# bolcom/serenade

Measured on AMD Instinct MI355X. Metric: predict_next queries/sec, higher is better.
Workload: dtype u32 ids / i32 accumulators / f64 scores; 1 GPU; BASELINE configs[2]: synthetic 60000000 interactions / 1760000 items, k=1500 m=2500 idf_weighting=2 last_items=4 how_many=21; batch_per_gpu=1048576, query_pool_batches=2, parallelism=query-sharded replicas x1 (no data-path collective), index=csr (built by this library)

## Files before the change

### serenade_amd/csrc/srn_fast.hip

```cpp
#include <hip/hip_runtime.h>

#include <cstdio>
#include <cstdlib>

#include "srn_device.h"
#include "srn_prep.h"
#include "srn_kernels.h"

namespace srn {

#ifndef SRN_FAST_NT
#define SRN_FAST_NT 1
#endif
typedef uint32_t fin_v4u __attribute__((ext_vector_type(4)));
__device__ __forceinline__ void fin_store(uint4* p, const uint4& v) {
#if SRN_FAST_NT
    __builtin_nontemporal_store((fin_v4u{v.x, v.y, v.z, v.w}), reinterpret_cast<fin_v4u*>(p));
#else
    *p = v;
#endif
}
__device__ __forceinline__ uint4 fin_load(const uint4* p) {
#if SRN_FAST_NT
    const fin_v4u v = __builtin_nontemporal_load(reinterpret_cast<const fin_v4u*>(p)); return make_uint4(v.x, v.y, v.z, v.w);
#else
    return *p;
#endif
}
template <typename T> __device__ __forceinline__ void row_store(T* p, T v) {
#if SRN_FAST_NT
    __builtin_nontemporal_store(v, p);
#else
    *p = v;
#endif
}

enum { FS_NB = 0, FS_FAIL, FS_SURV, FS_CCNT, FS_HITS, FS_LIVE, FS_SCAN_A = 8, FS_SCAN_B = 8, FS_W3 = 8, FS_CLS = 16, FS_TACC = 32 };
static constexpr uint32_t F_SIDF = F_LDS_BYTES, F_SATTR = F_SIDF + 512 * 8, F_TOTAL = F_SATTR + 512, F_SINV = F_W10 + 384;
static_assert(F_TOTAL * F_WG_PER_CU <= 160 * 1024, "LDS budget with the sample constants");

#ifndef SRN_FAST_RELOAD_ROWS
#define SRN_FAST_RELOAD_ROWS 0
#endif
#ifndef SRN_FAST_PRIO_LEVELS
#define SRN_FAST_PRIO_LEVELS 22201333
#endif
enum { FP_REC = 10000000, FP_FRONT = 1000000, FP_CUT = 100000, FP_REQ = 10000, FP_WALK = 1000, FP_HARV = 100, FP_WB = 10, FP_HAND = 1 };
#ifndef SRN_FAST_PRIO_X
#define SRN_FAST_PRIO_X 92
#endif
#define FAST_PRIO_X(div) do { if (SRN_FAST_PRIO_LEVELS && ((SRN_FAST_PRIO_X) / (div)) % 10 != 9) __builtin_amdgcn_s_setprio((short)(((SRN_FAST_PRIO_X) / (div)) % 10)); } while (0)
#ifndef SRN_MID_PRIO_LEVELS
#define SRN_MID_PRIO_LEVELS SRN_FAST_PRIO_LEVELS
#endif
#define FAST_PRIO(ph) do { if (SRN_FAST_PRIO_LEVELS) __builtin_amdgcn_s_setprio((short)((((MID) ? (SRN_MID_PRIO_LEVELS) : (SRN_FAST_PRIO_LEVELS)) / (ph)) % 10)); } while (0)
#ifndef SRN_FAST_STOP
#define SRN_FAST_STOP (-1)
#endif
#define FAST_TICK(ph) \
    do { if (ticking && tid == 0) { const long long t_ = clock64(); tacc[ph] += (unsigned long long)(t_ - t_prev); t_prev = t_; } } while (0); \
    if (SRN_FAST_STOP == (ph)) continue

__device__ __forceinline__ uint32_t fast_offset_of(uint32_t idx, uint64_t r) {
    if (idx < F_REP_ITEMS) return (F_DIRECT + idx * F_REP + ((uint32_t)r & (F_REP - 1u))) * 4u;
    return idx < F_DIRECT ? idx * 4u : (F_SKETCH - F_HOT) + (idx & (F_SK_WORDS - 1u)) * 4u;
}
#ifndef SRN_FAST_PHANTOM_OOR
#define SRN_FAST_PHANTOM_OOR 1
#endif
static constexpr uint32_t F_PHANTOM_WORDS = 256u;
static constexpr uint32_t F_PHANTOM = SRN_FAST_PHANTOM_OOR ? F_BIG_TOTAL - (F_TOTAL - F_SIDF) - 256u * 4u - F_M_MAX : F_DUMP;
static_assert(!SRN_FAST_PHANTOM_OOR || (F_PHANTOM >= F_TOTAL && F_PHANTOM % 4u == 0u), "the phantom words lie beyond the 53 KB forms' LDS allocation");
static_assert(F_PHANTOM + F_PHANTOM_WORDS * 4u - F_HOT <= 65536u, "16-bit row offsets");
static_assert(!SRN_FAST_PHANTOM_OOR || F_PHANTOM_WORDS * 4u <= F_M_MAX, "inside the numerator bytes' room");
__device__ __forceinline__ uint32_t fast_phantom(uint64_t r, uint32_t j) {
    return (F_PHANTOM - F_HOT) + ((((uint32_t)r * 0x9E3779B1u + j * 0x85EBCA6Bu) >> 21) & (F_PHANTOM_WORDS - 1u)) * 4u;
}
__global__ __launch_bounds__(1024) void rows_to_packed_kernel(const uint64_t* __restrict__ row_off, const uint32_t* __restrict__ row_items, uint64_t n,
                                                              const uint32_t* __restrict__ block_base, uint32_t* __restrict__ packed, uint32_t* __restrict__ ext16) {
    __shared__ uint32_t wave_tot[16];
    const uint64_t r = (uint64_t)blockIdx.x * 1024 + threadIdx.x;
    const int lane = threadIdx.x & 63, wave = threadIdx.x >> 6;
    uint64_t o = 0, len = 0;
    if (r < n) { o = row_off[r]; len = row_off[r + 1] - o; }
    const uint32_t e = len > 30 ? (uint32_t)((len - 28 + 7) / 8) : 0u;
    const uint32_t inc = wave_incl_scan(e);
    if (lane == 63) wave_tot[wave] = inc;
    __syncthreads();
    uint32_t base = block_base[blockIdx.x];
    for (int w = 0; w < wave; ++w) base += wave_tot[w];
    const uint32_t eblk = base + inc - e;
    if (r > n) return;
    const uint32_t inl = len > 30 ? 28u : (uint32_t)len;
    uint32_t sl[16];
    auto half = [&](uint32_t j) -> uint32_t { return j < inl ? fast_offset_of(row_items[o + j], r) : fast_phantom(r, j); };
    sl[0] = (uint32_t)(len > 0xFFFFu ? 0xFFFFu : len);
#pragma unroll
    for (uint32_t wd = 1; wd < 16; ++wd) sl[wd] = half(2 * wd - 2) | (half(2 * wd - 1) << 16);
    if (len > 30) {
        sl[15] = eblk;
        for (uint32_t b = 0; b < e; ++b) {
            uint32_t wv[4];
#pragma unroll
            for (uint32_t x = 0; x < 4; ++x) {
                const uint64_t j0 = 28 + 8ull * b + 2 * x;
                const uint32_t lo = j0 < len ? fast_offset_of(row_items[o + j0], r) : fast_phantom(r, (uint32_t)j0);
                const uint32_t hi = j0 + 1 < len ? fast_offset_of(row_items[o + j0 + 1], r) : fast_phantom(r, (uint32_t)j0 + 1);
                wv[x] = lo | (hi << 16);
            }
            reinterpret_cast<uint4*>(ext16)[(size_t)eblk + b] = make_uint4(wv[0], wv[1], wv[2], wv[3]);
        }
    }
    uint4* dst = reinterpret_cast<uint4*>(packed + r * 16);
#pragma unroll
    for (int qd = 0; qd < 4; ++qd) dst[qd] = make_uint4(sl[4 * qd], sl[4 * qd + 1], sl[4 * qd + 2], sl[4 * qd + 3]);
}

__global__ __launch_bounds__(1024) void rows_to_packed_frag_kernel(const uint64_t* __restrict__ row_off, const uint32_t* __restrict__ row_items, uint64_t n,
                                                                   const uint32_t* __restrict__ block_base, uint32_t* __restrict__ packed, uint32_t* __restrict__ ext16) {
    __shared__ uint32_t wave_tot[16];
    const uint64_t r = (uint64_t)blockIdx.x * 1024 + threadIdx.x;
    const int lane = threadIdx.x & 63, wave = threadIdx.x >> 6;
    uint64_t o = 0, len = 0;
    if (r < n) { o = row_off[r]; len = row_off[r + 1] - o; }
    const uint32_t e = len > 6 ? (uint32_t)((len - 4 + 7) / 8) : 0u;
    const uint32_t inc = wave_incl_scan(e);
    if (lane == 63) wave_tot[wave] = inc;
    __syncthreads();
    uint32_t base = block_base[blockIdx.x];
    for (int w = 0; w < wave; ++w) base += wave_tot[w];
    const uint32_t eblk = base + inc - e;
    if (r > n) return;
    const uint32_t inl = len > 6 ? 4u : (uint32_t)len;
    auto half = [&](uint32_t j) -> uint32_t { return j < inl ? fast_offset_of(row_items[o + j], r) : fast_phantom(r, j); };
    uint32_t sl[4];
    sl[0] = (uint32_t)(len > 0xFFFFu ? 0xFFFFu : len);
#pragma unroll
    for (uint32_t wd = 1; wd < 4; ++wd) sl[wd] = half(2 * wd - 2) | (half(2 * wd - 1) << 16);
    if (len > 6) {
        sl[3] = eblk;
        for (uint32_t b = 0; b < e; ++b) {
            uint32_t wv[4];
#pragma unroll
            for (uint32_t x = 0; x < 4; ++x) {
                const uint64_t j0 = 4 + 8ull * b + 2 * x;
                const uint32_t lo = j0 < len ? fast_offset_of(row_items[o + j0], r) : fast_phantom(r, (uint32_t)j0);
                const uint32_t hi = j0 + 1 < len ? fast_offset_of(row_items[o + j0 + 1], r) : fast_phantom(r, (uint32_t)j0 + 1);
                wv[x] = lo | (hi << 16);
            }
            reinterpret_cast<uint4*>(ext16)[(size_t)eblk + b] = make_uint4(wv[0], wv[1], wv[2], wv[3]);
        }
    }
    reinterpret_cast<uint4*>(packed)[r] = make_uint4(sl[0], sl[1], sl[2], sl[3]);
}

#ifndef SRN_MERGE_G
#define SRN_MERGE_G 8
#endif
__device__ __forceinline__ uint32_t merge_team(uint32_t total) {
    const uint32_t want = (total + (uint32_t)SRN_MERGE_G - 1u) / (uint32_t)SRN_MERGE_G;
    return want <= 64u ? 6u : want <= 128u ? 7u : want <= 256u ? 8u : 9u;
}
typedef __attribute__((address_space(3))) uint32_t lds_u32;
__device__ __forceinline__ uint32_t lds_addr(const uint32_t* p) { return (uint32_t)(uintptr_t)(const lds_u32*)p; }
__device__ __forceinline__ uint32_t lds_ld(uint32_t a) { return *(const lds_u32*)(uintptr_t)a; }
__device__ __forceinline__ void lds_st(uint32_t a, uint32_t v) { *(lds_u32*)(uintptr_t)a = v; }
__device__ __forceinline__ void merge_pair(const uint32_t* in, uint32_t* out, uint32_t sa, uint32_t la, uint32_t lb, uint32_t ttid, uint32_t lg_nthr) {
    if ((ttid >> lg_nthr) != 0u) return;
#ifndef SRN_MERGE_ODD
#define SRN_MERGE_ODD 1
#endif
    const uint32_t total = la + lb, g = ((total + (1u << lg_nthr) - 1u) >> lg_nthr) | (SRN_MERGE_ODD ? 1u : 0u);
    const uint32_t d0 = min(ttid * g, total), d1 = min(d0 + g, total);
    if (d0 >= d1) return;
    const uint32_t a0 = lds_addr(in) + sa * 4u;
    const uint32_t lo = d0 > lb ? d0 - lb : 0u, hi = min(d0, la);
    uint32_t p = a0 + lo * 4u - 4u;
    const uint32_t span = min(la, lb);
    if (span != 0u) {
        uint32_t xh = a0 + max(hi, 1u) * 4u - 4u, kb = d0 != 0u ? 2u * a0 + (la + d0) * 4u - 4u : 2u * a0;
        asm volatile("" : "+v"(xh), "+v"(kb));
        for (uint32_t st = 4u << (31u - (uint32_t)__clz((int)span)); st >= 4u; st >>= 1) {
            const uint32_t x = min(p + st, xh);
            p = lds_ld(x) > lds_ld(kb - x) ? x : p;
        }
    }
    uint32_t pa = p + 4u, pb = 2u * a0 + (la + d0) * 4u - 4u - p;
    uint32_t ea = a0 + la * 4u, eb = ea + lb * 4u;
    asm volatile("" : "+v"(ea), "+v"(eb));
    uint32_t va = 0u, vb = 0u;
    if (pa < ea) va = lds_ld(pa);
    if (pb < eb) vb = lds_ld(pb);
    uint32_t c = lds_addr(out) + (sa + d0) * 4u; const uint32_t ce = c + (d1 - d0) * 4u, ce1 = ce - 4u;
    auto put = [&](uint32_t off) {
        const bool ta = va > vb;
        lds_st(c + off, max(va, vb));
        const uint32_t q = (ta ? pa : pb) + 4u;
        pa = ta ? q : pa; pb = ta ? pb : q;
        const uint32_t nxt = lds_ld(q);
        const uint32_t nv = q < (ta ? ea : eb) ? nxt : 0u;
        va = ta ? nv : va; vb = ta ? vb : nv;
    };
    for (; c < ce1; c += 8u) { put(0u); put(4u); }
    if (c < ce) lds_st(c, max(va, vb));
}

#ifndef SRN_FAST_FUSED_CUT
#define SRN_FAST_FUSED_CUT 1
#endif
template <int G>
__device__ __forceinline__ uint32_t fast_cut(const uint32_t* F, uint32_t* nbl, uint32_t n, uint32_t NB, uint32_t m, uint32_t k, const uint8_t* wlut, uint32_t* misc, uint32_t tid, uint32_t lane) {
    constexpr int BLOCK = 512;
    const uint32_t NBM = (1u << NB) - 1u;
    const uint32_t g = (n + BLOCK - 1) / BLOCK, o0 = min(tid * g, n), o1 = min(o0 + g, n);
    uint32_t fv[G + 3];
#pragma unroll
    for (int x = 0; x < G + 3; ++x) fv[x] = F[min(o0 + (uint32_t)x, n - 1u)];
    const uint32_t prev0 = o0 > 0u && o0 < o1 ? F[o0 - 1u] >> NB : 0xFFFFFFFFu;
#pragma unroll
    for (int x = 0; x < G + 3; ++x) fv[x] = o0 + (uint32_t)x < n ? fv[x] : 0u;
    {
        uint32_t carry = 0u, carry_r = 0xFFFFFFFFu;
#pragma unroll
        for (int x = G + 2; x >= 0; --x) { const uint32_t r = fv[x] >> NB; carry = r == carry_r ? carry | fv[x] : fv[x]; carry_r = r; fv[x] = carry; }
    }
    uint32_t fmask = 0u, firsts = 0u;
    {
        uint32_t prev = prev0;
#pragma unroll
        for (int x = 0; x < G; ++x) { const bool in = o0 + (uint32_t)x < o1; const uint32_t r = fv[x] >> NB; const bool f1 = in && r != prev; fmask |= f1 ? 1u << x : 0u; firsts += f1; prev = in ? r : prev; }
    }
    uint32_t Call;
    const uint32_t idx0 = block_excl_scan<BLOCK>(firsts, misc + FS_SCAN_A, Call);
    const uint32_t Cm = min(Call, m);
    if (Cm <= k) {
        uint32_t idx = idx0;
#pragma unroll
        for (int x = 0; x < G; ++x) if ((fmask >> x) & 1u) { if (idx < m) nbl[idx] = fv[x]; ++idx; }
        return Cm;
    }
    uint32_t inm = 0u; unsigned long long nmp = 0ull, acc = 0ull;
    {
        uint32_t idx = idx0, nmv[G];
#pragma unroll
        for (int x = 0; x < G; ++x) nmv[x] = (uint32_t)wlut[fv[x] & NBM];
#pragma unroll
        for (int x = 0; x < G; ++x) {
            const bool f1 = (fmask >> x) & 1u, in = f1 && idx < m;
            idx += f1;
            inm |= in ? 1u << x : 0u;
            nmp |= in ? (unsigned long long)nmv[x] << (4 * x) : 0ull;
            acc += in ? 1ull << (4u * nmv[x]) : 0ull;
        }
    }
    uint32_t* cls = misc + FS_CLS;
    {
        const uint32_t wc = wave_class_counts(acc, lane);
        const uint32_t mycnt = lane < 16u ? wc : 0u;
        if (mycnt) atomicAdd(&cls[lane], mycnt);
    }
    __syncthreads();
    uint32_t nstar, rstar;
    {
        const uint32_t cv = lane < 16u ? cls[lane] : 0u; const uint32_t pre = wave_incl_scan(cv);
        const uint32_t suf = (uint32_t)__builtin_amdgcn_readlane((int)pre, 63) - pre + cv;
        const unsigned long long reach = __ballot(suf >= k);
        nstar = 63u - (uint32_t)__clzll((long long)reach);
        rstar = k - ((uint32_t)__builtin_amdgcn_readlane((int)suf, (int)nstar) - (uint32_t)__builtin_amdgcn_readlane((int)cv, (int)nstar));
    }
    uint32_t mine = 0;
#pragma unroll
    for (int x = 0; x < G; ++x) mine += ((inm >> x) & 1u) && (uint32_t)((nmp >> (4 * x)) & 15ull) == nstar;
    uint32_t tot_star;
    uint32_t before = block_excl_scan<BLOCK>(mine, misc + FS_SCAN_B, tot_star);
    uint32_t sel = 0, tmask = 0;
#pragma unroll
    for (int x = 0; x < G; ++x) {
        const bool in = (inm >> x) & 1u; const uint32_t c = (uint32_t)((nmp >> (4 * x)) & 15ull);
        const bool eq = in && c == nstar, take = in && (c > nstar || (eq && before < rstar));
        tmask |= take ? 1u << x : 0u; sel += take; before += eq;
    }
    const uint32_t inc = wave_incl_scan(sel);
    uint32_t base = 0; if (lane == 63u && inc) base = atomicAdd(&misc[FS_NB], inc);
    uint32_t at = (uint32_t)__builtin_amdgcn_readlane((int)base, 63) + inc - sel;
#pragma unroll
    for (int x = 0; x < G; ++x) if ((tmask >> x) & 1u) nbl[at++] = fv[x];
    return 0xFFFFFFFFu;
}

enum { FM_FUSED = 0, FM_FRONT = 1, FM_BACK = 2 };
template <int WG_PER_CU, bool FRAG, bool WIDE, int MODE = FM_FUSED, bool MID = false, bool BIG = false, bool LONG = false, bool TINY = false>
#ifndef SRN_FAST_WAVES
#define SRN_FAST_WAVES (WG_PER_CU * 2)
#endif
#ifndef SRN_TINY_WAVES
#define SRN_TINY_WAVES 2
#endif
__global__ __launch_bounds__(512, TINY ? SRN_TINY_WAVES : BIG ? 4 : SRN_FAST_WAVES) void vmis_fast_kernel(DeviceIndex ix_arg, LaunchParams p_arg, FastParams f_arg) {
#if SRN_FAST_SMALL
    static_assert(!BIG || MID, "BIG is a form of MID"); static_assert(!LONG || BIG, "LONG is a form of BIG");
    constexpr uint32_t SIDF = BIG ? F_BIG_TOTAL - (F_TOTAL - F_SIDF) : F_SIDF, SATTR = SIDF + 512 * 8;
    constexpr uint32_t MW = (SIDF - F_WORK) / 4;
    __shared__ __attribute__((aligned(16))) char smem[BIG ? F_BIG_TOTAL : F_TOTAL];
#else
    extern __shared__ __attribute__((aligned(16))) char smem[];
#endif
    typedef const __attribute__((address_space(4))) char* KArg;
    const KArg ka = (KArg)__builtin_amdgcn_kernarg_segment_ptr();
    constexpr size_t OFF_P = (sizeof(DeviceIndex) + alignof(LaunchParams) - 1) / alignof(LaunchParams) * alignof(LaunchParams);
    constexpr size_t OFF_F = (OFF_P + sizeof(LaunchParams) + alignof(FastParams) - 1) / alignof(FastParams) * alignof(FastParams);
    const __attribute__((address_space(4))) DeviceIndex& ix = *(const __attribute__((address_space(4))) DeviceIndex*)ka;
    const __attribute__((address_space(4))) LaunchParams& p = *(const __attribute__((address_space(4))) LaunchParams*)(ka + OFF_P);
    const __attribute__((address_space(4))) FastParams& f = *(const __attribute__((address_space(4))) FastParams*)(ka + OFF_F);
    constexpr int BLOCK = 512, NW = 8;
    constexpr int NL = LONG ? (int)F_LONG_LISTS : MID ? (int)F_MID_LISTS : 4;
    constexpr uint32_t SINV = F_SINV;
    static_assert(!MID || MODE == FM_FUSED, "MID: fused form only");
    const uint32_t tid = threadIdx.x, lane = tid & 63u, wave = tid >> 6;
    const unsigned long long lt = (1ull << lane) - 1ull;
// ... 347 lines not shown
            } else
                for (uint32_t o = o0; o < o1; ++o) { const uint32_t r = F[o] >> NB; firsts += r != prev; prev = r; }
            for (uint32_t i = tid; i < min(n, p.m); i += BLOCK) D[i] = 0;
            if (MID && tid < (LONG ? 256u : 64u)) cls_area[tid] = 0u;
            if constexpr (LONG) for (uint32_t i = tid; i < (min(n, p.m) + 3u) / 4u; i += BLOCK) dn_area[i] = 0u;
            uint32_t idx = block_excl_scan<BLOCK>(firsts, misc + FS_SCAN_A, Call);
            prev = prev0;
            if (g <= (uint32_t)MC_G) {
                uint32_t fv[MC_G];
#pragma unroll
                for (int x = 0; x < MC_G; ++x) fv[x] = F[min(o0 + (uint32_t)x, n - 1u)];
#pragma unroll
                for (int x = 0; x < MC_G; ++x) {
                    const bool in = o0 + (uint32_t)x < o1; const uint32_t r = fv[x] >> NB; const bool f1 = in && r != prev;
                    idx += f1; prev = in ? r : prev;
                    if constexpr (LONG) {
                        if (in && idx - 1u < p.m) { if (f1) D[idx - 1u] = fv[x]; atomicAdd(&dn_area[(idx - 1u) >> 2], (uint32_t)wlut[fv[x] & 31u] << (8u * ((idx - 1u) & 3u))); }
                    } else
                    if (in && idx - 1u < p.m) atomicOr(&D[idx - 1u], fv[x]);
                }
            } else
                for (uint32_t o = o0; o < o1; ++o) {
                    const uint32_t v = F[o], r = v >> NB; const bool f1 = r != prev;
                    idx += f1; prev = r;
                    if constexpr (LONG) { if (idx - 1u < p.m) { if (f1) D[idx - 1u] = v; atomicAdd(&dn_area[(idx - 1u) >> 2], (uint32_t)wlut[v & 31u] << (8u * ((idx - 1u) & 3u))); } }
                    else
                    if (idx - 1u < p.m) atomicOr(&D[idx - 1u], v);
                }
            Cm = min(Call, p.m);
        }
        __syncthreads();
        FAST_TICK(2);
        auto dn_of = [&](uint32_t i) -> uint32_t { return (dn_area[i >> 2] >> (8u * (i & 3u))) & 255u; };
        auto w_long = [&](uint32_t slot, uint32_t num) -> uint32_t { return (uint32_t)((9 - (int)(uint32_t)wlut[32u + (slot & 31u)]) * (int)num); };
        if (Cm <= p.k) {
            K = Cm;
            if constexpr (LONG) { for (uint32_t i = tid; i < Cm; i += BLOCK) { const uint32_t dvv = D[i]; nb2[i] = make_uint2(dvv, w_long(dvv, dn_of(i))); } __syncthreads(); }
        } else {
            uint32_t* cls = MID ? cls_area : misc + FS_CLS;
            const uint32_t g = (Cm + BLOCK - 1) / BLOCK, o0 = min(tid * g, Cm), o1 = min(o0 + g, Cm);
            uint32_t dv[5], nmv[5];
#pragma unroll
            for (int x = 0; x < 5; ++x) dv[x] = o0 + x < o1 ? D[o0 + x] : 0u;
#pragma unroll
            for (int x = 0; x < 5; ++x) { if constexpr (LONG) nmv[x] = o0 + x < o1 ? dn_of(o0 + (uint32_t)x) : 0u; else nmv[x] = o0 + x < o1 ? num_of(dv[x] & NBM) : 0u; }
            if constexpr (MID) {
#pragma unroll
                for (int x = 0; x < 5; ++x) if (o0 + x < o1) atomicAdd(&cls[nmv[x]], 1u);
            } else
            {
                unsigned long long acc = 0;
#pragma unroll
                for (int x = 0; x < 5; ++x) acc += o0 + x < o1 ? 1ull << (4u * nmv[x]) : 0ull;
                const uint32_t wc = wave_class_counts(acc, lane);
                const uint32_t mycnt = lane < 16u ? wc : 0u;
                if (mycnt) atomicAdd(&cls[lane], mycnt);
            }
            __syncthreads();
            uint32_t nstar, rstar;
            if constexpr (LONG) {
                const uint4 c4 = reinterpret_cast<const uint4*>(cls)[lane];
                const uint32_t s4 = c4.x + c4.y + c4.z + c4.w, pre4 = wave_incl_scan(s4);
                const uint32_t above = (uint32_t)__builtin_amdgcn_readlane((int)pre4, 63) - pre4;
                const uint32_t suf3 = above + c4.w, suf2 = suf3 + c4.z, suf1 = suf2 + c4.y, suf0 = suf1 + c4.x;
                const unsigned long long reach = __ballot(suf0 >= p.k);
                const int top = 63 - __clzll((long long)reach);
                const uint32_t jsel = suf3 >= p.k ? 3u : suf2 >= p.k ? 2u : suf1 >= p.k ? 1u : 0u;
                const uint32_t sufs = jsel == 3u ? suf3 : jsel == 2u ? suf2 : jsel == 1u ? suf1 : suf0, cnts = jsel == 3u ? c4.w : jsel == 2u ? c4.z : jsel == 1u ? c4.y : c4.x;
                nstar = (uint32_t)__builtin_amdgcn_readlane((int)(4u * lane + jsel), top);
                rstar = p.k - ((uint32_t)__builtin_amdgcn_readlane((int)sufs, top) - (uint32_t)__builtin_amdgcn_readlane((int)cnts, top));
            } else
            {
                const uint32_t cv = (MID || lane < 16u) ? cls[lane] : 0u; const uint32_t pre = wave_incl_scan(cv);
                const uint32_t suf = (uint32_t)__builtin_amdgcn_readlane((int)pre, 63) - pre + cv;
                const unsigned long long reach = __ballot(suf >= p.k);
                nstar = 63u - (uint32_t)__clzll((long long)reach);
                rstar = p.k - ((uint32_t)__builtin_amdgcn_readlane((int)suf, (int)nstar) - (uint32_t)__builtin_amdgcn_readlane((int)cv, (int)nstar));
            }
            uint32_t mine = 0;
#pragma unroll
            for (int x = 0; x < 5; ++x) mine += o0 + x < o1 && nmv[x] == nstar;
            uint32_t tot_star;
            uint32_t before = block_excl_scan<BLOCK>(mine, misc + FS_SCAN_B, tot_star);
            uint32_t sel = 0; bool take[5];
#pragma unroll
            for (int x = 0; x < 5; ++x) {
                const bool in_r = o0 + x < o1, eq = nmv[x] == nstar;
                take[x] = in_r && (nmv[x] > nstar || (eq && before < rstar));
                sel += take[x]; before += in_r && eq;
            }
            const uint32_t inc = wave_incl_scan(sel);
            uint32_t base = 0; if (lane == 63u && inc) base = atomicAdd(&misc[FS_NB], inc);
            uint32_t at = (uint32_t)__builtin_amdgcn_readlane((int)base, 63) + inc - sel;
#pragma unroll
            for (int x = 0; x < 5; ++x) if (take[x]) { if constexpr (LONG) nb2[at++] = make_uint2(dv[x], w_long(dv[x], nmv[x])); else nbl[at++] = dv[x]; }
            __syncthreads();
            K = misc[FS_NB];
        }
        }
        }

        FAST_TICK(4);
        if constexpr (SRN_FAST_ROW_PREFETCH == 2 && !MID && MODE == FM_FUSED && !FRAG) asm volatile("" :: "v"(pfv[0]), "v"(pfv[1]), "v"(pfv[2]), "v"(pfv[3]));
        FAST_PRIO(FP_REQ); FAST_PRIO_X(10);
        if constexpr (MODE == FM_FRONT) {
            if (tid == 0) xq[0] = K;
#pragma unroll
            for (int j = 0; j < 3; ++j) { const uint32_t e = tid + (uint32_t)j * BLOCK; if ((uint32_t)j * BLOCK < K && e < K) xq[1u + e] = nbl[e]; }
            continue;
        }

        uint32_t svr[3]; uint4 rq[3], rq1[3];
        uint32_t wvr[3] = {0u, 0u, 0u};
#pragma unroll
        for (int t = 0; t < 3; ++t) {
            const uint32_t j = wave * 64u + lane + (uint32_t)t * BLOCK;
            if constexpr (MODE == FM_BACK) svr[t] = j < K ? xsv[t] : 0u;
            else if constexpr (LONG) { const uint2 e2 = nb2[K ? min(j, K - 1u) : 0u]; svr[t] = K ? e2.x : 0u; wvr[t] = e2.y; }
            else
            svr[t] = K ? nbl[min(j, K - 1u)] : 0u;
            const size_t r = (MODE == FM_BACK ? j < K : K != 0u) ? (size_t)(base + (svr[t] >> NB)) : (size_t)n_kept;
            rq[t] = *reinterpret_cast<const uint4*>(&f.row_packed[r * (FRAG ? 1 : 4)]); rq1[t] = make_uint4(0u, 0u, 0u, 0u);
        }
        if (((SRN_FAST_PRIO_X) / 10) % 10 != 9) FAST_PRIO(FP_REQ);
        {
            uint4* z = reinterpret_cast<uint4*>(smem + F_HOT);
            for (uint32_t i = tid; i < (clr_lo - F_HOT) / 16u; i += BLOCK) z[i] = make_uint4(0u, 0u, 0u, 0u);
            if (tid < 64u) reinterpret_cast<uint4*>(thist)[tid] = make_uint4(0u, 0u, 0u, 0u);
            if (tid < F_TABLE_WORDS / 4u) { reinterpret_cast<uint4*>(ikeys)[tid] = make_uint4(EMPTY32, EMPTY32, EMPTY32, EMPTY32);
                                            reinterpret_cast<uint4*>(iacc)[tid] = make_uint4(0u, 0u, 0u, 0u); }
        }
        __syncthreads();
        FAST_PRIO(FP_WALK);
        FAST_TICK(8);
        auto add2 = [&](uint32_t wd, uint32_t w) {
            if constexpr (LONG) {
                const bool neg = (int)w < 0; const uint32_t a = wd & 0xFFFFu, b = wd >> 16;
                if (!neg || a < F_SKETCH - F_HOT) atomicAdd((uint32_t*)(acc_base + a), w);
                if (!neg || b < F_SKETCH - F_HOT) atomicAdd((uint32_t*)(acc_base + b), w);
            } else {
            atomicAdd((uint32_t*)(acc_base + (wd & 0xFFFFu)), w); atomicAdd((uint32_t*)(acc_base + (wd >> 16)), w); } };
        constexpr uint32_t INL1 = FRAG ? 6u : 14u, INL2 = FRAG ? 20u : 28u;
        uint32_t cnt3 = 0;
#pragma unroll
        for (int t = 0; t < 3; ++t) {
            const bool m3 = wave * 64u + lane + (uint32_t)t * BLOCK < K && (rq[t].x & 0xFFFFu) > INL1;
            const unsigned long long b3 = __ballot(m3);
            if (m3) nbl[qpos(cnt3 + (uint32_t)__popcll(b3 & lt))] = LONG ? wave * 64u + lane + (uint32_t)t * BLOCK : svr[t];
            cnt3 += (uint32_t)__popcll(b3);
        }
#ifdef SRN_FAST_SUBTICKS
        FAST_TICK(5);
#endif
        if constexpr (!FRAG) {
#pragma unroll
            for (int t = 0; t < 3; ++t) {
                const bool more6 = wave * 64u + lane + (uint32_t)t * BLOCK < K && (rq[t].x & 0xFFFFu) > 6u;
                const size_t r1 = more6 ? (size_t)(base + (svr[t] >> NB)) : (size_t)n_kept;
                rq1[t] = *reinterpret_cast<const uint4*>(&f.row_packed[r1 * 4 + 1]);
            }
        }
        auto tok_slot = [&](uint32_t tok) -> uint32_t { if constexpr (LONG) return nb2[tok].x; else return tok; };
        auto tok_w = [&](uint32_t tok, uint32_t slot) -> uint32_t { if constexpr (LONG) return nb2[tok].y; else return w10_of(slot & NBM); };
        auto q3_load = [&](uint32_t p0, uint32_t& tok, uint32_t& sv, uint32_t& hdr, uint4& c4, uint4& d4, uint32_t& blk) {
            tok = nbl[qpos(min(p0 + lane, cnt3 - 1u))];
            sv = tok_slot(tok);
            if constexpr (FRAG) {
                const uint4 s4 = *reinterpret_cast<const uint4*>(f.row_packed + (size_t)(base + (sv >> NB)));
                hdr = s4.x;
                const uint4* eb = reinterpret_cast<const uint4*>(f.row_ext16) + ((hdr & 0xFFFFu) > 6u ? (size_t)s4.w : (size_t)0);
                c4 = eb[0]; d4 = eb[1]; blk = s4.w + 2u;
            } else {
                const RowQuad* rowp = f.row_packed + (size_t)(base + (sv >> NB)) * 4;
                hdr = *reinterpret_cast<const uint32_t*>(rowp); c4 = *reinterpret_cast<const uint4*>(rowp + 2); d4 = *reinterpret_cast<const uint4*>(rowp + 3); blk = d4.w;
            } };
        uint32_t tk3 = 0, sv3 = 0, hdr3 = 0, blk3 = 0; uint4 c43 = make_uint4(0u, 0u, 0u, 0u), d43 = c43;
        if (cnt3) q3_load(0u, tk3, sv3, hdr3, c43, d43, blk3);
        const uint32_t qn = MID ? q_after : ordered || listed ? q_ord_next : q + gridDim.x;
        const bool park = MID ? q_after != 0xFFFFFFFFu : ordered || listed ? q_ord_next != 0xFFFFFFFFu : qn < p.nq;
        if (wave == 1u && park) {
            const char* const rn = p.prep + (size_t)qn * p.prep_stride + lane * 4u;
            if (lane * 4u < p.prep_stride) __builtin_amdgcn_global_load_lds((const __attribute__((address_space(1))) void*)rn, (__attribute__((address_space(3))) void*)pre, 4, 0, 0);
            if (256u + lane * 4u < min(p.prep_stride, 320u)) __builtin_amdgcn_global_load_lds((const __attribute__((address_space(1))) void*)(rn + 256), (__attribute__((address_space(3))) void*)(pre + 64), 4, 0, 0);
        }
#pragma unroll
        for (int t = 0; t < 3; ++t) {
            if (wave * 64u + (uint32_t)t * BLOCK < K) {
                const bool act = wave * 64u + lane + (uint32_t)t * BLOCK < K;
                const uint32_t w = LONG ? wvr[t] : w10_of(svr[t] & NBM), len = rq[t].x & 0xFFFFu;
                if constexpr (FRAG) { if (act) { add2(rq[t].y, w); add2(rq[t].z, w); if (len <= 6u) add2(rq[t].w, w); } }
                else {
                if (act) { add2(rq[t].y, w); add2(rq[t].z, w); add2(rq[t].w, w); }
                if (act && len > 6u) { add2(rq1[t].x, w); add2(rq1[t].y, w); add2(rq1[t].z, w); add2(rq1[t].w, w); }
                }
            }
        }
        auto add_tail = [&](uint32_t p0, uint32_t tok, uint32_t sv, uint32_t hdr, const uint4& c4, const uint4& d4, uint32_t blk) {
            const bool act = p0 + lane < cnt3;
            const uint32_t len = hdr & 0xFFFFu, w = tok_w(tok, sv);
            const bool more = FRAG ? true : len > 30u;
            if constexpr (FRAG) {
                if (act) { add2(c4.x, w); add2(c4.y, w); add2(c4.z, w); add2(c4.w, w); }
                if (act && len > 12u) { add2(d4.x, w); add2(d4.y, w); add2(d4.z, w); add2(d4.w, w); }
            } else if (act) {
                add2(c4.x, w); add2(c4.y, w); add2(c4.z, w); add2(c4.w, w);
                add2(d4.x, w); add2(d4.y, w); add2(d4.z, w);
                if (len <= 30u) add2(d4.w, w);
            }
            for (uint32_t t8 = INL2; __ballot(act && more && t8 < len) != 0ull; t8 += 8u) {
                if (act && more && t8 < len) {
                    const uint4 e4 = reinterpret_cast<const uint4*>(f.row_ext16)[(size_t)blk + ((t8 - INL2) >> 3)];
                    add2(e4.x, w); add2(e4.y, w); add2(e4.z, w); add2(e4.w, w);
                }
            } };
#ifdef SRN_FAST_SUBTICKS
        FAST_TICK(6);
#endif
        FAST_PRIO_X(1);
        if (cnt3) add_tail(0u, tk3, sv3, hdr3, c43, d43, blk3);
        for (uint32_t p0 = 64u; p0 < cnt3; p0 += 64u) { uint32_t tk, sv, hdr, blk; uint4 c4, d4; q3_load(p0, tk, sv, hdr, c4, d4, blk); add_tail(p0, tk, sv, hdr, c4, d4, blk); }
#ifdef SRN_FAST_SUBTICKS
        FAST_TICK(7);
#endif
        __syncthreads();
        FAST_PRIO(FP_HARV);
        FAST_TICK(9);
        uint32_t t32m1; uint32_t floor_b;
        {
            const uint32_t e = lane * NW + wave;
            uint32_t v = hot[e];
            if (F_REP_ITEMS && e < F_REP_ITEMS) {
                const uint4* rp = reinterpret_cast<const uint4*>(hot + F_DIRECT + e * F_REP);
                const uint4 a = rp[0], b = rp[1];
                v = a.x + a.y + a.z + a.w + b.x + b.y + b.z + b.w;
            }
            if (!SRN_FAST_PHANTOM_OOR || BIG)
            for (uint32_t i = tid; i < F_PHANTOM_WORDS; i += BLOCK) ((uint32_t*)(smem + F_PHANTOM))[i] = 0u;
            bool valid = (LONG ? (int)v > 0 : v != 0u) && e != cur_idx;
            double x = 0.0; uint32_t tie = 0;
            tie = f.meta_sample[tid].id_rank;
            if (business) valid = valid && business_ok(cur_attr, (uint32_t)((const uint8_t*)(smem + SATTR))[tid]);
            if (valid) x = ((const double*)(smem + SIDF))[tid] * (double)v;
            const uint32_t k32 = (uint32_t)((unsigned long long)__double_as_longlong(x) >> 32);
            {
                uint32_t vv = k32, third = 0;
#pragma unroll
                for (int t = 0; t < 3; ++t) {
                    const uint32_t mx = wave_max(vv);
                    third = mx;
                    const unsigned long long bal = __ballot(vv == mx);
                    if ((int)lane == __ffsll((long long)bal) - 1) vv = 0;
                }
                for (uint32_t t = 3u; t < ((p.how_many + 7u) >> 3); ++t) {
                    const uint32_t mx = wave_max(vv);
                    third = mx;
                    const unsigned long long bal = __ballot(vv == mx);
                    if ((int)lane == __ffsll((long long)bal) - 1) vv = 0;
                }
                if (lane == 0u) misc[FS_W3 + wave] = third;
            }
            __syncthreads();
            uint32_t t32 = 0xFFFFFFFFu;
#pragma unroll
            for (int w = 0; w < NW; ++w) t32 = min(t32, misc[FS_W3 + w]);
            t32m1 = t32 ? t32 - 1u : 0u;
            const bool take = valid && k32 >= t32m1;
            const uint32_t at = wave_append(take, &misc[FS_CCNT]);
            if (take) { if (at < F_CAND_CAP) { ckey[at] = (unsigned long long)__double_as_longlong(x); cidx[at] = tie; } else misc[FS_FAIL] = 1;
                        const uint32_t hb = k32 >> 16, tb = t32 >> 16; if (t32) atomicAdd(&thist[hb > tb ? min(hb - tb, 255u) : 0u], 1u); }
            const double x_lo = __longlong_as_double((long long)((unsigned long long)t32m1 << 32));
            const double inv = ((const double*)(smem + SINV))[min(lane, 8u)];
            const uint32_t my_floor = (uint32_t)fmin(4.0e9, fmax(1.0, floor(x_lo * inv * (1.0 - 1e-9)) - 1.0));
            floor_b = (uint32_t)__builtin_amdgcn_readlane((int)my_floor, 8);
            {
                const uint32_t wv = (uint32_t)__builtin_amdgcn_readfirstlane((int)wave);
                const uint4* h4 = reinterpret_cast<const uint4*>(hot);
                static_assert(F_HOT_WORDS == 4096 || F_HOT_WORDS == 3840, "quads per thread below (3840: the 40 KB timing experiment)");
                constexpr uint32_t NQ2 = F_HOT_WORDS / 4u - 128u - (uint32_t)BLOCK;
                const uint4 a4 = h4[128u + tid];
                const uint4 b4 = tid < NQ2 ? h4[128u + (uint32_t)BLOCK + tid] : make_uint4(0u, 0u, 0u, 0u);
                if (tid == NQ2 - 1u) hot[F_HOT_WORDS - 1u] = 0u;
                const uint32_t fl1 = (uint32_t)__builtin_amdgcn_readlane((int)my_floor, (int)(1u + (wv >> 1)));
                const uint32_t fl2 = (uint32_t)__builtin_amdgcn_readlane((int)my_floor, (int)min(5u + (wv >> 1), 7u));
                auto quad = [&](const uint4& q4, uint32_t e0, uint32_t fl) {
                    const uint32_t mx = LONG ? (uint32_t)max(max(max((int)q4.x, (int)q4.y), max((int)q4.z, (int)q4.w)), 0) : max(max(q4.x, q4.y), max(q4.z, q4.w));
                    if (__ballot(mx >= fl) == 0ull) return;
                    const uint32_t vv[4] = {q4.x, q4.y, q4.z, q4.w};
#pragma unroll
                    for (uint32_t j = 0; j < 4u; ++j) {
                        const uint32_t e2 = e0 + j;
                        const bool pass = (LONG ? (int)vv[j] >= (int)fl : vv[j] >= fl) && e2 != cur_idx && e2 < F_DIRECT;
                        const uint32_t at2 = wave_append(pass, &misc[FS_SURV]);
                        if (pass) { if (at2 < SURV_CAP && vv[j] < (1u << 20)) surv[at2] = (e2 << 20) | vv[j]; else atomicOr(&misc[FS_FAIL], 2u); }
                    } };
                quad(a4, 512u + 4u * tid, fl1);
                quad(b4, 512u + 4u * ((uint32_t)BLOCK + tid), fl2);
            }
        }
        __syncthreads();
        {
            const uint4 h4 = reinterpret_cast<const uint4*>(thist)[lane];
            const uint32_t sum4 = h4.x + h4.y + h4.z + h4.w, pre = wave_incl_scan(sum4);
            uint32_t above = (uint32_t)__builtin_amdgcn_readlane((int)pre, 63) - pre;
            const uint32_t need = p.how_many;
            const bool mine = above < need && need <= above + sum4;
            uint32_t bin = 4u * lane + 3u;
            if (above + h4.w < need) { above += h4.w; bin = 4u * lane + 2u;
                if (above + h4.z < need) { above += h4.z; bin = 4u * lane + 1u;
                    if (above + h4.y < need) bin = 4u * lane; } }
            const unsigned long long mb = __ballot(mine);
            const uint32_t bsel = mb ? (uint32_t)__builtin_amdgcn_readlane((int)bin, __ffsll((long long)mb) - 1) : 0u;
            if (bsel) {
                const uint32_t t32b = (((t32m1 + 1u) >> 16) + bsel) << 16;
                t32m1 = t32b - 1u;
                const double x_lo = __longlong_as_double((long long)((unsigned long long)t32m1 << 32));
                floor_b = (uint32_t)fmin(4.0e9, fmax(1.0, floor(x_lo * ((const double*)(smem + SINV))[8] * (1.0 - 1e-9)) - 1.0));
            }
        }
        if (wave == 1u) asm volatile("s_waitcnt vmcnt(0)" ::: "memory");
        FAST_TICK(10);
        FAST_PRIO(FP_WB);
        {
            const uint32_t ns = min(misc[FS_SURV], SURV_CAP);
            for (uint32_t i = tid; i < ns; i += BLOCK) {
                const uint32_t sv = surv[i], e = sv >> 20, v = sv & 0xFFFFFu;
                const ItemMeta mt = ix.meta[e];
                const double x = (mt.idf > 0.0 ? mt.idf : 1.0) * (double)v;
                const bool take = (uint32_t)((unsigned long long)__double_as_longlong(x) >> 32) >= t32m1 && (!business || business_ok(cur_attr, mt.attr));
                const uint32_t at = wave_append(take, &misc[FS_CCNT]);
                if (take) { if (at < F_CAND_CAP) { ckey[at] = (unsigned long long)__double_as_longlong(x); cidx[at] = mt.id_rank; } else misc[FS_FAIL] = 1; }
            }
        }
        {
            const uint4* sk4 = reinterpret_cast<const uint4*>(smem + F_SKETCH);
            uint32_t mx = 0;
            for (uint32_t i = tid; i < F_SK_WORDS / 4u; i += BLOCK) { const uint4 w4 = sk4[i]; mx = max(max(mx, w4.x), max(max(w4.y, w4.z), w4.w)); }
            if (__ballot(mx >= floor_b) != 0ull && lane == 0u) misc[FS_LIVE] = 1u;
        }
        __syncthreads();
        have_pre = park;
        const bool live = misc[FS_LIVE] != 0u;
        if (live) {
        {
            uint32_t dbg_hits = 0;
            auto chk2 = [&](uint32_t hm, uint32_t wd) -> uint32_t {
                const uint32_t a = *(const uint32_t*)(acc_base + max(wd & 0xFFFFu, F_ZERO_OFF)), b = *(const uint32_t*)(acc_base + max(wd >> 16, F_ZERO_OFF));
                return (hm << 2) | (a >= floor_b ? 2u : 0u) | (b >= floor_b ? 1u : 0u); };
            auto list_hits = [&](uint32_t hm, uint32_t npos, uint32_t sv, uint32_t j0) {
                const uint32_t c = (uint32_t)__popc(hm);
                if (__ballot(c != 0u) == 0ull) return;
                dbg_hits += c;
                const uint32_t inc = wave_incl_scan(c);
                uint32_t base = 0; if (lane == 63u) base = atomicAdd(&misc[FS_HITS], inc);
                uint32_t at = (uint32_t)__builtin_amdgcn_readlane((int)base, 63) + inc - c;
                while (hm) {
                    const uint32_t b = 31u - (uint32_t)__clz((int)hm); hm &= ~(1u << b);
                    if (at < F_HIT_CAP) hits[at] = make_uint2(sv, j0 + (npos - 1u - b)); else atomicOr(&misc[FS_FAIL], 4u);
                    ++at;
                }
            };
            auto mx2 = [&](uint32_t mx, uint32_t wd) -> uint32_t {
                const uint32_t a = *(const uint32_t*)(acc_base + max(wd & 0xFFFFu, F_ZERO_OFF)), b = *(const uint32_t*)(acc_base + max(wd >> 16, F_ZERO_OFF));
                return max(max(mx, a), b); };
            uint32_t tk3b = 0, sv3b = 0, hdr3b = 0, blk3b = 0; uint4 c43b = make_uint4(0u, 0u, 0u, 0u), d43b = c43b;
#if SRN_FAST_RELOAD_ROWS
#pragma unroll
            for (int t = 0; t < 3; ++t) {
                const size_t r = K ? (size_t)(base + (svr[t] >> NB)) : (size_t)n_kept;
                rq[t] = *reinterpret_cast<const uint4*>(&f.row_packed[r * 4]);
                rq1[t] = *reinterpret_cast<const uint4*>(&f.row_packed[r * 4 + 1]);
            }
#endif
            if (cnt3) q3_load(0u, tk3b, sv3b, hdr3b, c43b, d43b, blk3b);
#pragma unroll
            for (int t = 0; t < 3; ++t) {
                if (wave * 64u + (uint32_t)t * BLOCK < K) {
                    const bool act = wave * 64u + lane + (uint32_t)t * BLOCK < K, two = (rq[t].x & 0xFFFFu) > 6u;
                    uint32_t mx = 0;
                    if constexpr (FRAG) {
                        if (act) { mx = mx2(mx2(0u, rq[t].y), rq[t].z); if (!two) mx = mx2(mx, rq[t].w); }
                        if (__ballot(mx >= floor_b) != 0ull) {
                            uint32_t hm = 0;
                            if (act) { hm = chk2(chk2(0u, rq[t].y), rq[t].z); hm = two ? hm << 2 : chk2(hm, rq[t].w); }
                            list_hits(hm, 6u, LONG ? wave * 64u + lane + (uint32_t)t * BLOCK : svr[t], 0u);
                        }
                    } else {
                    if (act) { mx = mx2(mx2(mx2(0u, rq[t].y), rq[t].z), rq[t].w); if (two) mx = mx2(mx2(mx2(mx2(mx, rq1[t].x), rq1[t].y), rq1[t].z), rq1[t].w); }
                    if (__ballot(mx >= floor_b) != 0ull) {
                        uint32_t hm = 0;
                        if (act) {
                            hm = chk2(chk2(chk2(0u, rq[t].y), rq[t].z), rq[t].w) << 8;
                            if (two) hm = chk2(chk2(chk2(chk2(hm >> 8, rq1[t].x), rq1[t].y), rq1[t].z), rq1[t].w);
                        }
                        list_hits(hm, 14u, LONG ? wave * 64u + lane + (uint32_t)t * BLOCK : svr[t], 0u);
                    }
                    }
                }
            }
            auto chk_tail = [&](uint32_t p0, uint32_t sv, uint32_t hdr, const uint4& c4, const uint4& d4, uint32_t blk) {
                const bool act = p0 + lane < cnt3;
                const uint32_t len = hdr & 0xFFFFu;
                const bool more = FRAG ? true : len > 30u;
                uint32_t hm = 0, mx = 0;
                if constexpr (FRAG) {
                    const bool two = len > 12u;
                    if (act) { mx = mx2(mx2(mx2(mx2(0u, c4.x), c4.y), c4.z), c4.w); if (two) mx = mx2(mx2(mx2(mx2(mx, d4.x), d4.y), d4.z), d4.w); }
                    if (__ballot(mx >= floor_b) != 0ull) {
                        uint32_t hmd = 0;
                        if (act) { hm = chk2(chk2(chk2(chk2(0u, c4.x), c4.y), c4.z), c4.w); if (two) hmd = chk2(chk2(chk2(chk2(0u, d4.x), d4.y), d4.z), d4.w); }
                        list_hits(hm, 8u, sv, 4u); list_hits(hmd, 8u, sv, 12u);
                    }
                } else {
                if (act) { mx = mx2(mx2(mx2(mx2(mx2(mx2(mx2(0u, c4.x), c4.y), c4.z), c4.w), d4.x), d4.y), d4.z); if (len <= 30u) mx = mx2(mx, d4.w); }
                if (__ballot(mx >= floor_b) != 0ull) {
                if (act) {
                    hm = chk2(chk2(chk2(chk2(chk2(chk2(chk2(0u, c4.x), c4.y), c4.z), c4.w), d4.x), d4.y), d4.z);
                    if (len > 30u) hm <<= 2; else hm = chk2(hm, d4.w);
                }
                list_hits(hm, 16u, sv, 14u); }
                }
                for (uint32_t t8 = INL2; __ballot(act && more && t8 < len) != 0ull; t8 += 8u) {
                    uint32_t hm2 = 0;
                    if (act && more && t8 < len) {
                        const uint4 e4 = reinterpret_cast<const uint4*>(f.row_ext16)[(size_t)blk + ((t8 - INL2) >> 3)];
                        hm2 = chk2(chk2(chk2(chk2(0u, e4.x), e4.y), e4.z), e4.w);
                    }
                    list_hits(hm2, 8u, sv, t8);
                } };
            if (cnt3) chk_tail(0u, tk3b, hdr3b, c43b, d43b, blk3b);
            for (uint32_t p0 = 64u; p0 < cnt3; p0 += 64u) { uint32_t tk, sv, hdr, blk; uint4 c4, d4; q3_load(p0, tk, sv, hdr, c4, d4, blk); chk_tail(p0, tk, hdr, c4, d4, blk); }
            if (ticking) { const uint32_t hs = wave_sum(dbg_hits); if (lane == 0u && hs) atomicAdd(&tacc[5], (unsigned long long)hs); }
        }
        __syncthreads();
        FAST_TICK(11);
        {
            const uint32_t nh = min(misc[FS_HITS], F_HIT_CAP);
            if (ticking && tid == 0 && nh == 0u) tacc[7] += 1ull;
            bool ovf = false;
            for (uint32_t i = tid; i < nh; i += BLOCK) {
                const uint2 h = hits[i];
                const uint32_t hslot = tok_slot(h.x);
                const uint32_t* os = reinterpret_cast<const uint32_t*>(ix.row_slots + (size_t)(base + (hslot >> NB)) * (FRAG ? 1 : 4));
                const uint32_t len = os[0], j = h.y;
                uint32_t it = EMPTY32;
                if constexpr (FRAG) { if (j < len) it = len <= 3u ? os[1 + j] : (j < 2u ? os[2 + j] : ix.row_ext[os[1] + (j - 2u)]); }
                else
                if (j < len) it = len <= 15u ? os[1 + j] : (j < 14u ? os[2 + j] : ix.row_ext[os[1] + (j - 14u)]);
                if (business && it != EMPTY32 && it >= F_DIRECT && !business_ok(cur_attr, ix.meta[it].attr)) it = EMPTY32;
                if (it != EMPTY32 && it >= F_DIRECT && item_insert(ikeys, iacc, F_TABLE_BUCKETS, it, (int)tok_w(h.x, hslot)) < 0) ovf = true;
            }
            if (ovf) atomicOr(&misc[FS_FAIL], 8u);
        }
        __syncthreads();
        }
        FAST_TICK(12);
        if (misc[FS_FAIL]) {
            if (tid == 0) { f.slow_list[atomicAdd(&f.slow_cnt[SC_GENERAL], 1u)] = q; if (ticking) { const uint32_t c = misc[FS_FAIL]; tacc[15] += (c & 1u) + ((unsigned long long)((c >> 1) & 1u) << 16) + ((unsigned long long)((c >> 2) & 1u) << 32) + ((unsigned long long)((c >> 3) & 1u) << 48); } }
            continue;
        }
        if (wave != 0u) continue;
        FAST_PRIO(FP_HAND);
        uint32_t ln = lane; asm volatile("" : "+v"(ln));
        const unsigned long long ltl = (1ull << ln) - 1ull;
        uint2* tl = hits;
        uint32_t nt = 0;
        if (live)
#pragma unroll
        for (uint32_t b0 = 0; b0 < (F_TABLE_BUCKETS + 63u) / 64u; ++b0) {
            const uint32_t bk = b0 * 64u + ln;
            uint4 kq = make_uint4(EMPTY32, EMPTY32, EMPTY32, EMPTY32), aq = make_uint4(0u, 0u, 0u, 0u);
            if (bk < F_TABLE_BUCKETS) { kq = reinterpret_cast<const uint4*>(ikeys)[bk]; aq = reinterpret_cast<const uint4*>(iacc)[bk]; }
            const uint32_t kk[4] = {kq.x, kq.y, kq.z, kq.w}, aa[4] = {aq.x, aq.y, aq.z, aq.w};
#pragma unroll
            for (int s4 = 0; s4 < 4; ++s4) {
                const bool in = kk[s4] != EMPTY32 && kk[s4] != cur_idx && (LONG ? (int)aa[s4] >= (int)floor_b : aa[s4] >= floor_b);
                const unsigned long long bm = __ballot(in);
                if (in) tl[nt + (uint32_t)__popcll(bm & ltl)] = make_uint2(kk[s4], aa[s4]);
                nt += (uint32_t)__popcll(bm);
            }
        }
        uint32_t cnt = misc[FS_CCNT];
        if (cnt + nt > F_FIN_ENTRIES && cnt <= F_CAND_CAP) {
            unsigned long long xs[3]; uint32_t ti[3];
#pragma unroll
            for (uint32_t t = 0; t < 3u; ++t) { const uint32_t i = t * 64u + ln; xs[t] = i < cnt ? ckey[i] : 0ull; ti[t] = i < cnt ? cidx[i] : 0u; }
            uint32_t c2 = 0;
#pragma unroll
            for (uint32_t t = 0; t < 3u; ++t) {
                const bool keep = t * 64u + ln < cnt && (uint32_t)(xs[t] >> 32) >= t32m1;
                const unsigned long long bm = __ballot(keep);
                if (keep) { const uint32_t at = c2 + (uint32_t)__popcll(bm & ltl); ckey[at] = xs[t]; cidx[at] = ti[t]; }
                c2 += (uint32_t)__popcll(bm);
            }
            cnt = c2;
        }
        const uint32_t M = cnt + nt;
        if (MID && (LONG || L == 10u) && M < p.how_many) {
            if (ln == 0u) f.slow_list[atomicAdd(&f.slow_cnt[SC_GENERAL], 1u)] = q;
            continue;
        }
        if constexpr (TINY) {
            constexpr uint32_t TB_MAX = 704, TB_SLOTS = TB_MAX / 64;
            static_assert(F_CAND_CAP + 4u * F_TABLE_BUCKETS <= TB_MAX && TB_MAX * 12u + 64u * 12u <= F_SK_WORDS * 4u, "the big row's keys fit the sketch words");
            if (M > F_FIN_ENTRIES && M <= TB_MAX && cnt <= F_CAND_CAP && M >= p.how_many) {
                unsigned long long* const kx = reinterpret_cast<unsigned long long*>(smem + F_SKETCH); uint32_t* const kt = reinterpret_cast<uint32_t*>(smem + F_SKETCH + TB_MAX * 8u);
                unsigned long long* const cx = reinterpret_cast<unsigned long long*>(smem + F_SKETCH + TB_MAX * 12u); uint32_t* const ct = reinterpret_cast<uint32_t*>(smem + F_SKETCH + TB_MAX * 12u + 64u * 8u);
                uint32_t hk[TB_SLOTS];
                {
                    uint2 cc[TB_SLOTS]; ItemMeta mm[TB_SLOTS];
#pragma unroll
                    for (uint32_t t = 0; t < TB_SLOTS; ++t) { const uint32_t i = t * 64u + ln; cc[t] = i >= cnt && i < M ? tl[i - cnt] : make_uint2(0u, 0u); }
#pragma unroll
                    for (uint32_t t = 0; t < TB_SLOTS; ++t) mm[t] = ix.meta[cc[t].x];
#pragma unroll
                    for (uint32_t t = 0; t < TB_SLOTS; ++t) {
                        const uint32_t i = t * 64u + ln;
                        unsigned long long x = 0ull; uint32_t tie = EMPTY32;
                        if (i < cnt) { x = ckey[i]; tie = cidx[i]; }
                        else if (i < M) { x = (unsigned long long)__double_as_longlong((mm[t].idf > 0.0 ? mm[t].idf : 1.0) * (double)cc[t].y); tie = mm[t].id_rank; }
                        hk[t] = (uint32_t)(x >> 32);
                        if (i < M) { kx[i] = x; kt[i] = tie; }
                    }
                }
                uint32_t t32 = 0u;
                for (int b = 31; b >= 0; --b) {
                    const uint32_t c = t32 | (1u << b);
                    uint32_t n_ge = 0;
#pragma unroll
                    for (uint32_t t = 0; t < TB_SLOTS; ++t) n_ge += (uint32_t)__popcll(__ballot(hk[t] >= c));
                    t32 = n_ge >= p.how_many ? c : t32;
                }
                const uint32_t cut = t32 ? t32 - 1u : 0u;
                uint32_t S = 0;
#pragma unroll
                for (uint32_t t = 0; t < TB_SLOTS; ++t) {
                    const uint32_t i = t * 64u + ln;
                    const bool keep = i < M && hk[t] >= cut && hk[t] != 0u;
                    const unsigned long long bm = __ballot(keep);
                    const uint32_t at = S + (uint32_t)__popcll(bm & ltl);
                    if (keep && at < 64u) { cx[at] = kx[i]; ct[at] = kt[i]; }
                    S += (uint32_t)__popcll(bm);
                }
                if (S <= 64u && S >= p.how_many) {
                    __builtin_amdgcn_wave_barrier();
                    uint4 e = make_uint4(0u, 0u, 0u, 0u);
                    if (ln < S) { const unsigned long long x = cx[ln]; e = make_uint4((uint32_t)x, (uint32_t)(x >> 32), ct[ln], 0u); }
                    finish_inline(ix_arg, S, U, e, ln, q, p.out_ids, p.out_scores, p.out_counts, p.how_many);
                    continue;
                }
            }
        }
        uint32_t ovf_at = 0;
        if (M > F_FIN_ENTRIES) {
            unsigned long long tk = 0;
            if (ln == 0u) tk = atomicAdd(f.big_ticket, (1ull << 32) | (unsigned long long)(M - F_FIN_ENTRIES));
            const uint32_t slot = (uint32_t)__builtin_amdgcn_readlane((int)(uint32_t)(tk >> 32), 0);
            ovf_at = (uint32_t)__builtin_amdgcn_readlane((int)(uint32_t)tk, 0);
            if (cnt > F_CAND_CAP || (unsigned long long)ovf_at + (M - F_FIN_ENTRIES) > f.big_cap_entries) {
                if (ln == 0u) { f.big_list[slot] = 0xFFFFFFFFu; f.slow_list[atomicAdd(&f.slow_cnt[SC_GENERAL], 1u)] = q; }
                continue;
            }
            if (ln == 0u) f.big_list[slot] = q;
        }
        if constexpr (TINY) {
            if (M <= F_FIN_ENTRIES) {
                uint4 e = make_uint4(0u, 0u, 0u, 0u);
                if (ln < cnt) { const unsigned long long x = ckey[ln]; e = make_uint4((uint32_t)x, (uint32_t)(x >> 32), cidx[ln], 0u); }
                else if (ln < M) { const uint2 c = tl[ln - cnt]; e = make_uint4(c.y, 0u, c.x, 1u); }
                finish_inline(ix_arg, M, U, e, ln, q, p.out_ids, p.out_scores, p.out_counts, p.how_many);
                continue;
            }
        }
        {
            uint4* rec = reinterpret_cast<uint4*>(f.fin + (size_t)q * F_FIN_BYTES);
            uint4* ovf = reinterpret_cast<uint4*>(f.big_arena) + ovf_at;
            if (ln == 0u) { fin_store(&rec[0], make_uint4(M, U, ovf_at, 0u)); p.out_counts[q] = M > F_FIN_ENTRIES ? 0x80000001u : 0x80000000u; }
#ifdef SRN_FAST_EXP_NOHANDOFF
            for (uint32_t i = ln; i < 0u; i += 64u) {
#else
            for (uint32_t i = ln; i < M; i += 64u) {
#endif
                uint4 e;
                if (i < cnt) { const unsigned long long x = ckey[i]; e = make_uint4((uint32_t)x, (uint32_t)(x >> 32), cidx[i], 0u); }
// ... 246 lines not shown
```

Measured before the change: 55.43 million queries/s.

## Reorder fast-path loads to overlap prefetch with scatter adds via uncounted LDS loads

Issues the next-query prefetch with an inline-asm global_load_lds that sets M0 directly, so the compiler does not insert vmcnt waits that stall the following atomic adds. Precomputes neighbour weights and the first tail weight before the prefetch. Splits the short- and long-row add loops so the first part runs before the rq1 loads are needed, and defers reading blk from d4 behind an asm barrier to move register dependencies later. This adds risk: the inline asm bypasses the compiler's tracking of load counters and M0.

Measured after the change: 56.20 million queries/s (median of 6 runs). 1.4% higher.

```diff
diff --git a/serenade_amd/csrc/srn_fast.hip b/serenade_amd/csrc/srn_fast.hip
--- a/serenade_amd/csrc/srn_fast.hip
+++ b/serenade_amd/csrc/srn_fast.hip
@@ -57,8 +57,11 @@
 #ifndef SRN_FAST_STOP
 #define SRN_FAST_STOP (-1)
 #endif
+#ifndef SRN_FAST_TICK_TID
+#define SRN_FAST_TICK_TID 0
+#endif
 #define FAST_TICK(ph) \
-    do { if (ticking && tid == 0) { const long long t_ = clock64(); tacc[ph] += (unsigned long long)(t_ - t_prev); t_prev = t_; } } while (0); \
+    do { if (ticking && tid == (SRN_FAST_TICK_TID)) { const long long t_ = clock64(); tacc[ph] += (unsigned long long)(t_ - t_prev); t_prev = t_; } } while (0); \
     if (SRN_FAST_STOP == (ph)) continue
 
 __device__ __forceinline__ uint32_t fast_offset_of(uint32_t idx, uint64_t r) {
@@ -165,6 +168,10 @@
 __device__ __forceinline__ uint32_t lds_addr(const uint32_t* p) { return (uint32_t)(uintptr_t)(const lds_u32*)p; }
 __device__ __forceinline__ uint32_t lds_ld(uint32_t a) { return *(const lds_u32*)(uintptr_t)a; }
 __device__ __forceinline__ void lds_st(uint32_t a, uint32_t v) { *(lds_u32*)(uintptr_t)a = v; }
+__device__ __forceinline__ void glds_dword_uncounted(const void* g, uint32_t dst) {
+    uint32_t keep;
+    asm volatile("s_mov_b32 %0, m0\n\ts_mov_b32 m0, %2\n\ts_nop 0\n\tglobal_load_lds_dword %1, off\n\ts_mov_b32 m0, %0" : "=&s"(keep) : "v"(g), "s"(dst) : "memory");
+}
 __device__ __forceinline__ void merge_pair(const uint32_t* in, uint32_t* out, uint32_t sa, uint32_t la, uint32_t lb, uint32_t ttid, uint32_t lg_nthr) {
     if ((ttid >> lg_nthr) != 0u) return;
 #ifndef SRN_MERGE_ODD
@@ -818,6 +825,9 @@
 #ifdef SRN_FAST_SUBTICKS
         FAST_TICK(5);
 #endif
+        uint32_t wr[3];
+#pragma unroll
+        for (int t = 0; t < 3; ++t) wr[t] = LONG ? wvr[t] : w10_of(svr[t] & NBM);
         if constexpr (!FRAG) {
 #pragma unroll
             for (int t = 0; t < 3; ++t) {
@@ -838,32 +848,41 @@
                 c4 = eb[0]; d4 = eb[1]; blk = s4.w + 2u;
             } else {
                 const RowQuad* rowp = f.row_packed + (size_t)(base + (sv >> NB)) * 4;
-                hdr = *reinterpret_cast<const uint32_t*>(rowp); c4 = *reinterpret_cast<const uint4*>(rowp + 2); d4 = *reinterpret_cast<const uint4*>(rowp + 3); blk = d4.w;
+                hdr = *reinterpret_cast<const uint32_t*>(rowp); c4 = *reinterpret_cast<const uint4*>(rowp + 2); d4 = *reinterpret_cast<const uint4*>(rowp + 3); blk = 0u;
             } };
         uint32_t tk3 = 0, sv3 = 0, hdr3 = 0, blk3 = 0; uint4 c43 = make_uint4(0u, 0u, 0u, 0u), d43 = c43;
         if (cnt3) q3_load(0u, tk3, sv3, hdr3, c43, d43, blk3);
+        const uint32_t w3 = cnt3 ? tok_w(tk3, sv3) : 0u;
         const uint32_t qn = MID ? q_after : ordered || listed ? q_ord_next : q + gridDim.x;
         const bool park = MID ? q_after != 0xFFFFFFFFu : ordered || listed ? q_ord_next != 0xFFFFFFFFu : qn < p.nq;
         if (wave == 1u && park) {
             const char* const rn = p.prep + (size_t)qn * p.prep_stride + lane * 4u;
-            if (lane * 4u < p.prep_stride) __builtin_amdgcn_global_load_lds((const __attribute__((address_space(1))) void*)rn, (__attribute__((address_space(3))) void*)pre, 4, 0, 0);
-            if (256u + lane * 4u < min(p.prep_stride, 320u)) __builtin_amdgcn_global_load_lds((const __attribute__((address_space(1))) void*)(rn + 256), (__attribute__((address_space(3))) void*)(pre + 64), 4, 0, 0);
+            const uint32_t dst = (uint32_t)__builtin_amdgcn_readfirstlane((int)lds_addr(pre));
+            if (lane * 4u < p.prep_stride) glds_dword_uncounted(rn, dst);
+            if (256u + lane * 4u < min(p.prep_stride, 320u)) glds_dword_uncounted(rn + 256, dst + 256u);
         }
 #pragma unroll
         for (int t = 0; t < 3; ++t) {
             if (wave * 64u + (uint32_t)t * BLOCK < K) {
                 const bool act = wave * 64u + lane + (uint32_t)t * BLOCK < K;
-                const uint32_t w = LONG ? wvr[t] : w10_of(svr[t] & NBM), len = rq[t].x & 0xFFFFu;
+                const uint32_t w = wr[t], len = rq[t].x & 0xFFFFu;
                 if constexpr (FRAG) { if (act) { add2(rq[t].y, w); add2(rq[t].z, w); if (len <= 6u) add2(rq[t].w, w); } }
-                else {
-                if (act) { add2(rq[t].y, w); add2(rq[t].z, w); add2(rq[t].w, w); }
+                else if (act) { add2(rq[t].y, w); add2(rq[t].z, w); add2(rq[t].w, w); }
+            }
+        }
+        if constexpr (!FRAG) {
+#pragma unroll
+        for (int t = 0; t < 3; ++t) {
+            if (wave * 64u + (uint32_t)t * BLOCK < K) {
+                const bool act = wave * 64u + lane + (uint32_t)t * BLOCK < K;
+                const uint32_t w = wr[t], len = rq[t].x & 0xFFFFu;
                 if (act && len > 6u) { add2(rq1[t].x, w); add2(rq1[t].y, w); add2(rq1[t].z, w); add2(rq1[t].w, w); }
-                }
-            }
-        }
-        auto add_tail = [&](uint32_t p0, uint32_t tok, uint32_t sv, uint32_t hdr, const uint4& c4, const uint4& d4, uint32_t blk) {
+            }
+        }
+        }
+        auto add_tail = [&](uint32_t p0, uint32_t w, uint32_t hdr, const uint4& c4, const uint4& d4, uint32_t blk) {
             const bool act = p0 + lane < cnt3;
-            const uint32_t len = hdr & 0xFFFFu, w = tok_w(tok, sv);
+            const uint32_t len = hdr & 0xFFFFu;
             const bool more = FRAG ? true : len > 30u;
             if constexpr (FRAG) {
                 if (act) { add2(c4.x, w); add2(c4.y, w); add2(c4.z, w); add2(c4.w, w); }
@@ -883,8 +902,12 @@
         FAST_TICK(6);
 #endif
         FAST_PRIO_X(1);
-        if (cnt3) add_tail(0u, tk3, sv3, hdr3, c43, d43, blk3);
-        for (uint32_t p0 = 64u; p0 < cnt3; p0 += 64u) { uint32_t tk, sv, hdr, blk; uint4 c4, d4; q3_load(p0, tk, sv, hdr, c4, d4, blk); add_tail(p0, tk, sv, hdr, c4, d4, blk); }
+        { fin_v4u dv = {d43.x, d43.y, d43.z, d43.w};
+          asm volatile("" : "+v"(hdr3), "+v"(dv));
+          d43 = make_uint4(dv.x, dv.y, dv.z, dv.w); }
+        if constexpr (!FRAG) blk3 = d43.w;
+        if (cnt3) add_tail(0u, w3, hdr3, c43, d43, blk3);
+        for (uint32_t p0 = 64u; p0 < cnt3; p0 += 64u) { uint32_t tk, sv, hdr, blk; uint4 c4, d4; q3_load(p0, tk, sv, hdr, c4, d4, blk); if constexpr (!FRAG) blk = d4.w; add_tail(p0, tok_w(tk, sv), hdr, c4, d4, blk); }
 #ifdef SRN_FAST_SUBTICKS
         FAST_TICK(7);
 #endif
@@ -1038,6 +1061,7 @@
             }
 #endif
             if (cnt3) q3_load(0u, tk3b, sv3b, hdr3b, c43b, d43b, blk3b);
+            if constexpr (!FRAG) blk3b = d43b.w;
 #pragma unroll
             for (int t = 0; t < 3; ++t) {
                 if (wave * 64u + (uint32_t)t * BLOCK < K) {
@@ -1094,7 +1118,7 @@
                     list_hits(hm2, 8u, sv, t8);
                 } };
             if (cnt3) chk_tail(0u, tk3b, hdr3b, c43b, d43b, blk3b);
-            for (uint32_t p0 = 64u; p0 < cnt3; p0 += 64u) { uint32_t tk, sv, hdr, blk; uint4 c4, d4; q3_load(p0, tk, sv, hdr, c4, d4, blk); chk_tail(p0, tk, hdr, c4, d4, blk); }
+            for (uint32_t p0 = 64u; p0 < cnt3; p0 += 64u) { uint32_t tk, sv, hdr, blk; uint4 c4, d4; q3_load(p0, tk, sv, hdr, c4, d4, blk); if constexpr (!FRAG) blk = d4.w; chk_tail(p0, tk, hdr, c4, d4, blk); }
             if (ticking) { const uint32_t hs = wave_sum(dbg_hits); if (lane == 0u && hs) atomicAdd(&tacc[5], (unsigned long long)hs); }
         }
         __syncthreads();
```
